# AlgoLab/RecGraph

Hardware: AMD Instinct MI355X
Metric: aligned reads/sec (-m 8 recombination, 1 kbp reads, 10k-row/32-path graph) (higher is better)
Workload: dtype int16

## Files before the change

### recgraph_amd/csrc/rg_host.hpp

```cpp
#pragma once
#include "rg_codes.hpp"

#include <atomic>
#include <cstdint>
#include <deque>
#include <functional>
#include <string>
#include <vector>

#include "../../include/recgraph_hip.h"

namespace rg {

extern thread_local std::string g_last_error;

#define RG_OPTIONS(X) \
    X(sweep_i32, "RG_SWEEP_I32", B, 0, 1, 0)           \
    X(three_sweeps, "RG_THREE_SWEEPS", B, 0, 1, 0)     \
    X(no_frec, "RG_NO_FREC", B, 0, 1, 0)               \
    X(debug, "RG_DEBUG", B, 0, 1, 0)                   \
    X(spin_wait, "RG_SPIN_WAIT", B, 0, 1, 0)           \
    X(no_gather, "RG_NO_GATHER", B, 0, 1, 0)           \
    X(no_split, "RG_NO_SPLIT", B, 0, 1, 0)             \
    X(no_spec, "RG_NO_SPEC", B, 0, 1, 0)               \
    X(spec_margin, "RG_SPEC_MARGIN", I, -(1 << 24), 1 << 24, 112)    \
    X(spec4_margin_x10, "RG_SPEC4_MARGIN_X10", I, 0, 1000, 25)       \
    X(stripe_c, "RG_STRIPE_C", I, 0, 32, 0)            \
    X(no_retire, "RG_NO_RETIRE", I, 0, 3, 0)           \
    X(retire_shift, "RG_RETIRE_SHIFT", I, 2, 12, RG_SWEEP16_RETIRE_SHIFT)    \
    X(no_order, "RG_NO_ORDER", B, 0, 1, 0)             \
    X(dsel_edge, "RG_DSEL_EDGE", I, 1, 1 << 20, 8)     \
    X(no_dsel, "RG_NO_DSEL", B, 0, 1, 0)               \
    X(no_pick2, "RG_NO_PICK2", B, 0, 1, 0)             \
    X(layer_i32, "RG_LAYER_I32", B, 0, 1, 0)           \
    X(lds_pad, "RG_LDS_PAD", I, 0, 40 << 10, 0)        \
    X(chunk_reads, "RG_CHUNK_READS", I, 0, 1 << 20, 0)    \
    X(launch_log, "RG_LAUNCH_LOG", B, 0, 1, 0)
struct Options {
#define RG_OPTION_FIELD(name, env, kind, lo, hi, def) std::atomic<int> name{def};
    RG_OPTIONS(RG_OPTION_FIELD)
#undef RG_OPTION_FIELD
};
struct OptionDesc {
    const char* name;
    const char* env;
    bool boolean;
    int lo, hi, def;
    std::atomic<int> Options::*slot;
};
extern const OptionDesc kOptionTable[];
extern const int kOptionCount;
const OptionDesc* find_option(const char* name);
void store_option(Options& o, const OptionDesc& d, long long value);
Options& options();
int wait_stream_sleeping(void* stream, void* ev, bool spin = false);

int fail(int code, const std::string& msg);

inline long long even_chunks(long long n, long long maxchunk) {
    const long long nchunks = (n + maxchunk - 1) / maxchunk;
    return (n + nchunks - 1) / nchunks;
}

// ... 135 lines not shown
```

### recgraph_amd/csrc/rg_kernel_timer.hpp

```cpp
#pragma once
#include <vector>

#include "rg_path_args.hpp"

namespace rg {

struct KernelTimer {
    hipStream_t stream = nullptr;
    bool spin = false;
    std::vector<hipEvent_t> ev;
    hipEvent_t done_ev = nullptr;
    std::vector<const char*> pend;
    std::vector<const char*> insts;

    KernelTimer() = default;
    KernelTimer(const KernelTimer&) = delete;
    ~KernelTimer() {
        for (auto e : ev) (void)hipEventDestroy(e);
        if (done_ev) (void)hipEventDestroy(done_ev);
    }
    void reset() { pend.clear(); insts.clear(); }
    int inst(const char* label, const char* what = "an untimed launch") {
        if (!label) return fail(RG_ERR_ARG, std::string("no kernel is compiled for this launch: ") + what);
        if (options().launch_log) insts.push_back(label);
        return RG_OK;
    }
    template <typename F>
    int run(const char* name, F&& launch) {
        const size_t used = 2 * pend.size();
        while (ev.size() < used + 2) {
            hipEvent_t e;
            HIPCHK(hipEventCreate(&e));
            ev.push_back(e);
        }
        HIPCHK(hipEventRecord(ev[used], stream));
        const char* label = launch();
        HIPCHK(hipGetLastError());
        HIPCHK(hipEventRecord(ev[used + 1], stream));
        pend.push_back(name);
        return inst(label, name);
    }
    int collect(KernelStats& stats) {
        if (!pend.empty()) {
            if (!done_ev) HIPCHK(hipEventCreateWithFlags(&done_ev, hipEventDisableTiming));
            HIPCHK((hipError_t)wait_stream_sleeping(stream, done_ev, spin));
            for (size_t k = 0; k < pend.size(); ++k) {
                float ms = 0;
                HIPCHK(hipEventElapsedTime(&ms, ev[2 * k], ev[2 * k + 1]));
                add_stat(stats, pend[k], ms, 1);
            }
            pend.clear();
        }
        for (const char* l : insts) add_stat(stats, std::string("inst:") + l, 0, 1);
        insts.clear();
        return RG_OK;
    }
};

}
```

### recgraph_amd/csrc/rg_path_driver.hip

```cpp
#include <algorithm>
#include <chrono>
#include <cstdio>
#include <cstdlib>
#include <cstring>

#include "gap/rg_path_gap.hpp"
#include "gap_local/rg_path_gap_local.hpp"
#include "rg_kernel_timer.hpp"
#include "rg_path_kernels.hpp"
#include "rg_path_plan.hpp"

namespace rg {

struct PathWorkImpl {
    bool tables = false;
    DevBuf<int> fpoff, fprow, fpslot, rpoff, rprow, rpslot;
    DevBuf<ReadState> state;
    DevBuf<int> roll, mf, wr, mfarg, wrarg, thr, flayer, rlayer;
    DevBuf<uint32_t> fdirs, rdirs, gdirs;
    DevBuf<Cand> fcand, rcand;
    DevBuf<unsigned> nf, nr, ridx, nrec, nrrec;
    DevBuf<int> frec, rrec;
    unsigned frec_cap = 0, rrec_cap = 0;
    DevBuf<int> lb;
// ... 299 lines not shown
        HIPCHK(hipMemsetAsync(w.nr.p, 0, sizeof(unsigned) * chunk, stream));
        ExpandArgs ea{w.state.p, w.frec.p, w.frec_cap, w.nrec.p, w.fcand.p, w.fcap, w.nf.p, w.wr.p, wpad, p.base_rec_cost, gd.knm, 0, off(), p.rec_band_width, p.scores[5]};
        RG_TRY(T.run("k_expand", [&] { return launch_expand(ea, chunk, plan.C, stream); }));
        ExpandArgs er{w.state.p, w.rrec.p, w.rrec_cap, w.nrrec.p, w.rcand.p, w.rcap, w.nr.p, w.mf.p, wpad, p.base_rec_cost, gd.knm, 1, off(), p.rec_band_width, p.scores[5]};
        RG_TRY(T.run("k_expand", [&] { return launch_expand(er, chunk, plan.C, stream); }));
    }
    SearchArgs sr{gd, w.state.p, w.fcand.p, w.rcand.p, w.nf.p, w.nr.p, w.ridx.p, w.fcap, w.rcap, w.wr.p, wpad, p.base_rec_cost, p.multi_rec_cost};
    RG_TRY(T.run("k_search", [&] { return launch_search(sr, chunk, stream); }));
    RG_TRY(T.inst(launch_need(w.state.p, w.nf.p, w.nr.p, plan.use_rec ? w.nrec.p : nullptr, plan.use_rec ? w.nrrec.p : nullptr, w.need.p, chunk, stream)));
    if (plan.spec) RG_TRY(T.inst(launch_verify(w.state.p, w.lb.p, w.need.p + 4, w.rt_flags.p, chunk, sa.dsel_pick, sa.dsel_pick2, sa.dsel_lo, sa.dsel_hi, stream)));
    return RG_OK;
}

int Run::enqueue_tail() {
    const int C = plan.C;
    LayerArgs la;
    memset(&la, 0, sizeof la);
    la.semi = plan.semi ? 1 : 0;
    la.nwv = plan.nwv;
    la.g = gd; la.sc = sc; la.reads = d_reads; la.read_off = off(); la.state = w.state.p; la.dir_words = plan.dir_words; la.dir_fmt = plan.use16 ? 1 : 0;
    la.layer_stride = plan.layer_stride; la.fpoff = w.fpoff.p; la.fprow = w.fprow.p; la.fpslot = w.fpslot.p;
    la.rpoff = w.rpoff.p; la.rprow = w.rprow.p; la.rpslot = w.rpslot.p;
    la.rev = 0; la.dirs = w.fdirs.p; la.dirs_stride = plan.fdirs_stride; la.layer = w.flayer.p;
    auto layer = [&]() { return plan.layer16 ? launch_layer16(la, chunk, C, stream) : launch_layer(la, chunk, C, stream); };
    RG_TRY(T.run("k_layer_fwd", layer));
    if (plan.mode == RG_MODE_RECOMBINATION) {
        la.rev = 1; la.dirs = w.rdirs.p; la.dirs_stride = plan.rdirs_stride; la.layer = w.rlayer.p;
        RG_TRY(T.run("k_layer_rev", layer));
    }
    TraceArgs ta;
    memset(&ta, 0, sizeof ta);
    ta.g = gd; ta.sc = sc; ta.reads = d_reads; ta.read_off = off(); ta.state = w.state.p; ta.rec = d_rec + done;
    ta.ops = d_ops + (long long)done * ops_stride; ta.ops_stride = ops_stride; ta.flayer = w.flayer.p;
    ta.rlayer = w.rlayer.p; ta.layer_stride = plan.layer_stride; ta.fpoff = w.fpoff.p; ta.fprow = w.fprow.p;
    ta.rpoff = w.rpoff.p; ta.rprow = w.rprow.p; ta.nreads = chunk; ta.mode = p.mode; ta.semi = plan.semi ? 1 : 0; ta.nwv = plan.nwv;
    RG_TRY(T.run("k_trace", [&] { return launch_trace(ta, C, stream); }));
    return read_back();
}

int Run::read_back() {
    HIPCHK(hipMemcpyAsync(w.h_sum, d_cells, sizeof(unsigned long long), hipMemcpyDeviceToHost, stream));
    HIPCHK(hipMemcpyAsync(w.h_sum + 5, d_cells + 1, sizeof(unsigned long long), hipMemcpyDeviceToHost, stream));
    HIPCHK(hipMemcpyAsync(w.h_sum + 1, w.need.p, 8 * sizeof(unsigned), hipMemcpyDeviceToHost, stream));
    return T.collect(stats);
}

int Run::enqueue_chunk() {
    HIPCHK(hipMemsetAsync(w.state.p, 0, sizeof(ReadState) * chunk, stream));
    if (plan.gap) return enqueue_pathwise_gap();
    SweepArgs sa = sweep_args();
    SeedArgs se;
    se.g = gd; se.state = w.state.p; se.nreads = chunk; se.mode = p.mode; se.sc = sc; se.reads = d_reads; se.read_off = off();
    int rc = plan.mode == RG_MODE_PATHWISE ? enqueue_pathwise(sa, se) : enqueue_recombination(sa, se);
    if (rc) return rc;
    return enqueue_tail();
}

int Run::dump_list_stats() {
    const unsigned* nd = need();
// ... 153 lines not shown
        const size_t per_read_all = plan.per_read_all(w.fcap, w.rcap, w.frec_cap, w.rrec_cap);
        int maxchunk = (int)std::min<size_t>(8192, std::max<size_t>(1, (budget >> oom_shift) / per_read_all));
        if (opt.chunk_reads > 0) maxchunk = std::min<int>(maxchunk, opt.chunk_reads);
        const double dbg_t0 = r.debug ? now_s() : 0;
        const int chunk = r.chunk = (int)even_chunks(nreads - r.done, maxchunk);
        bool oom = false;
        if ((rc = r.alloc_chunk(&oom))) {
            if (rc == RG_ERR_HIP && oom && chunk > 1 && oom_shift < 12) { ++oom_shift; continue; }
            return rc;
        }
        if (r.debug) fprintf(stderr, "[rg] chunk of %d reads: buffers ready after %.1f ms\n", chunk, (now_s() - dbg_t0) * 1e3);
        if ((rc = r.enqueue_chunk())) return rc;
        if (r.debug) fprintf(stderr, "[rg] chunk of %d reads: done after %.1f ms\n", chunk, (now_s() - dbg_t0) * 1e3);
        if (r.async_err != hipSuccess) return fail(RG_ERR_HIP, std::string("hipMemsetAsync: ") + hipGetErrorString(r.async_err));
        bool redo = false;
        if ((rc = r.regrow_lists(redo))) return rc;
        if (redo) continue;
        const unsigned long long chunk_cells = w.h_sum[0];
        cells_perf += w.h_sum[5];
        const unsigned nretry = r.nretry();
        if (r.debug && (plan.spec || plan.spec4)) fprintf(stderr, "[rg] speculative bound (margin %d): %u of %d reads did not reach it\n", plan.spec_margin, nretry, chunk);
        if (r.debug && plan.spec4 && nretry && (rc = r.dump_spec4_retries())) return rc;
        if (r.debug && plan.dsel && (rc = r.dump_dsel_retries())) return rc;
        if (nretry && (rc = r.second_pass(cells_perf))) return rc;
        cells_done += chunk_cells;
        r.done += chunk;
        add_stat(stats, "mem:work_bytes_per_read", (double)per_read_all, 1);
    }
    cells[0] += cells_done;
    cells[1] += cells_perf;
    return RG_OK;
}

}
```

### recgraph_amd/csrc/rg_path_kernels.hpp

```cpp
#pragma once
#include "rg_path_args.hpp"
#include "rg_path_plan.hpp"
#include "rg_launch_log.hpp"

namespace rg {

template <int H>
__device__ __forceinline__ void dir16_decode(unsigned w, unsigned& u16, unsigned& l16) {
    constexpr unsigned LOWH = (1u << H) - 1u;
    const unsigned t = __brev(w);
    u16 = ((t >> 24) & LOWH) | (((t >> 16) & LOWH) << H);
    l16 = ((t >> 8) & LOWH) | ((t & LOWH) << H);
}

struct SweepArgs {
    PathGraphDev g;
    DevScores sc;
    const uint8_t* reads;
    const long long* read_off;
    const uint8_t* bad;
    ReadState* state;
    int* roll;
    int rev;
    int track_best;
    const int* thr;
    const int4* fsteps;
// ... 127 lines not shown
    const int* wr;
    int wpad;
    int brc;
    float mrc;
};

struct LayerArgs {
    PathGraphDev g;
    DevScores sc;
    const uint8_t* reads;
    const long long* read_off;
    ReadState* state;
    int rev;
    const uint32_t* dirs;
    long long dirs_stride;
    int dir_words;
    int dir_fmt;
    int semi;
    int* layer;
    long long layer_stride;
    const int* fpoff; const int* fprow; const int* fpslot;
    const int* rpoff; const int* rprow; const int* rpslot;
    int nwv;
};

struct TraceArgs {
    PathGraphDev g;
    DevScores sc;
    const uint8_t* reads;
    const long long* read_off;
    ReadState* state;
    DevRecord* rec;
    uint8_t* ops;
    long long ops_stride;
    const int* flayer;
    const int* rlayer;
    long long layer_stride;
    const int* fpoff; const int* fprow;
    const int* rpoff; const int* rprow;
    int nreads;
    int mode;
    int semi;
    int nwv;
};

const char* launch_sweep(const SweepArgs& a, int nreads, int C, hipStream_t s);
const char* launch_sweep16(const SweepArgs& a, int nreads, int C, hipStream_t s);
const char* launch_expand(const ExpandArgs& a, int nreads, int C, hipStream_t s);
const char* launch_colmax_rec(const ExpandArgs& a, int* colmax_out, int* colarg_out, int nreads, int C, hipStream_t s);
const char* launch_seed(const SeedArgs& a, hipStream_t s);
const char* launch_opt0(const Opt0Args& a, int nreads, int C, hipStream_t s);
const char* launch_opt0_16(const Opt0Args& a, int nreads, int C, hipStream_t s);
const char* launch_pick(const PickArgs& a, int nreads, hipStream_t s);
const char* launch_order(const int* pick, const int* pick2, int* order, int nreads, hipStream_t s);
const char* launch_verify4(ReadState* st, const int* lb, unsigned* nretry, uint8_t* flags, int nreads, const int* dsel_pick, hipStream_t s);
const char* launch_verify(ReadState* st, const int* lb, unsigned* nretry, uint8_t* flags, int nreads, const int* dsel_pick, const int* dsel_pick2, int dsel_lo, int dsel_hi, hipStream_t s);
const char* launch_gather_reads(const uint8_t* reads, const long long* off, const int* idx, const long long* sub_off, uint8_t* out, int n, hipStream_t s);
const char* launch_scatter_results(const int* idx, const DevRecord* sub_rec, const uint8_t* sub_ops, DevRecord* rec, uint8_t* ops, long long ops_stride, int n, hipStream_t s);
const char* launch_threshold(const ThrArgs& a, int nreads, hipStream_t s);
const char* launch_bound(const BoundArgs& a, int nreads, hipStream_t s);
const char* launch_search(const SearchArgs& a, int nreads, hipStream_t s);
const char* launch_need(const ReadState* st, const unsigned* nf, const unsigned* nr, const unsigned* nrec, const unsigned* nrrec,
                 unsigned* need, int nreads, hipStream_t s);
const char* launch_layer(const LayerArgs& a, int nreads, int C, hipStream_t s);
const char* launch_layer16(const LayerArgs& a, int nreads, int C, hipStream_t s);
const char* launch_trace(const TraceArgs& a, int C, hipStream_t s);

}
```

### recgraph_amd/csrc/rg_path_plan.cpp

```cpp
#include "rg_path_plan.hpp"

#include <algorithm>
#include <climits>
#include <cmath>
#include <cstdlib>
#include <cstring>
#include <mutex>

namespace rg {

#define RG_OPTION_ROW(name, env, kind, lo, hi, def) {#name, env, #kind[0] == 'B', lo, hi, def, &Options::name},
const OptionDesc kOptionTable[] = {RG_OPTIONS(RG_OPTION_ROW)};
#undef RG_OPTION_ROW
const int kOptionCount = (int)(sizeof kOptionTable / sizeof kOptionTable[0]);

const OptionDesc* find_option(const char* name) {
    if (!name) return nullptr;
    for (const OptionDesc& d : kOptionTable)
        if (!strcmp(name, d.name)) return &d;
    return nullptr;
}
void store_option(Options& o, const OptionDesc& d, long long value) {
    o.*d.slot = d.boolean ? (value ? 1 : 0) : (int)std::max<long long>(d.lo, std::min<long long>(value, d.hi));
}
Options& options() {
    static Options o;
    static std::once_flag once;
    std::call_once(once, [] {
        for (const OptionDesc& d : kOptionTable) {
            const char* v = getenv(d.env);
            if (!v) continue;
            store_option(o, d, d.boolean ? (*v && strcmp(v, "0") != 0) : atoi(v));
        }
    });
    return o;
// ... 96 lines not shown
        o.gaps_nonpos = o.gaps_nonpos && p.scores[x * 6 + 5] <= 0 && p.scores[5 * 6 + x] <= 0;
        o.gaps_agree = o.gaps_agree && p.scores[5 * 6 + x] == p.scores[x * 6 + 5];
        for (int y = 0; y < 5; ++y) o.maxmatch = std::max(o.maxmatch, p.scores[x * 6 + y]);
    }
    o.two_sweep = recomb && o.gaps_nonpos && !opt.three_sweeps;
    o.use_rec = o.two_sweep && use16 && !opt.no_frec;
    const bool paths_ok = P <= 64 || use16;
    o.spec = o.two_sweep && spec_level < 2 && !semi && paths_ok && !opt.no_spec;
    o.score_scale = std::max(1, o.maxmatch / 2);
    const int per_kbp = (max_n + 999) / 1000;
    o.spec_margin = ((nwv > 1 ? opt.spec_margin * per_kbp : (int)opt.spec_margin) + (spec_level == 1 ? 320 * per_kbp : 0)) *
                    (opt.spec_margin > 0 ? o.score_scale : 1);
    o.pick_two = o.spec && !opt.no_pick2;
    o.dsel = o.spec && o.use_rec && spec_level == 0 && !opt.no_dsel;
    { const int e = L / std::max(1, (int)opt.dsel_edge); o.dsel_lo = e; o.dsel_hi = L - 1 - e; }
    o.rec_pen = p.base_rec_cost + (int)std::ceil(p.multi_rec_cost * 8.0f);
    o.spec4 = o.mode == RG_MODE_PATHWISE && !semi && use16 && o.gaps_nonpos && spec_level == 0 && !opt.no_spec;
    o.spec4_margin = o.spec_margin * opt.spec4_margin_x10 / 10;
    o.retire4 = o.spec4 && opt.no_retire != 1;
    o.dsel4 = o.spec4 && !opt.no_dsel;
    o.order = !opt.no_order;
    o.opt16 = use16;
    o.layer16 = use16 && o.gaps_agree && !opt.layer_i32;
    o.gather_ok = use16 && !opt.no_gather;
    o.use_split = o.gather_ok && !semi && C <= 16 && !opt.no_split;
    o.retire = (use16 || nwv == 1 || C <= 16) && paths_ok && !semi && recomb && o.gaps_nonpos && opt.no_retire != 1;
    o.retire_fwd = o.retire && opt.no_retire != 3;
    o.retire_rev = o.retire && opt.no_retire != 2;
    o.fcap = (o.two_sweep && !o.use_rec) ? 1u << 20 : 1u << 15;
    o.rcap = o.use_rec ? 1u << 16 : 1u << 19;
    o.frec_cap = o.spec ? 1u << 14 : 1u << 16;
    o.rrec_cap = o.spec ? 1u << 13 : 1u << 15;
    return RG_OK;
}

void build_path_rows(const HostGraph& h, bool fwd, std::vector<int>& poff, std::vector<int>& prow, std::vector<int>& pslot) {
    const std::vector<int32_t>& goff = fwd ? h.fgoff : h.rgoff;
    const std::vector<GroupDesc>& groups = fwd ? h.fgroups : h.rgroups;
    const int P = h.P, L = h.L;
    std::vector<std::vector<std::pair<int, int>>> per(P);
    for (int step = 1; step + 1 < L; ++step) {
        const int i = fwd ? step : L - 1 - step;
        for (int gi = goff[i]; gi < goff[i + 1]; ++gi)
            for (int b = 0; b < 64; ++b)
                if ((groups[gi].mask >> b) & 1) per[groups[gi].page * 64 + b].push_back({i, groups[gi].slot});
    }
// ... 40 lines not shown
```

### recgraph_amd/csrc/rg_path_plan.hpp

```cpp
#pragma once
#include <cstddef>
#include <vector>

#include "rg_host.hpp"

namespace rg {

struct ReadState {
    uint32_t status;
    int s0;
    int seed_path;
    int end_row;
    int end_row_best;
    int fwd_path, rev_path, fen, rsn, rec_col, displacement;
    float fscore;
    int bound;
    int sink_val[RG_MAXP];
    int trace_score;
    int path_end_row[RG_MAXP];
};

struct Cand {
    int row, col, val, path;
};

struct PathPlanInput {
    int P, L, fslots, rslots, max_path_rows, max_n;
};

struct PathPlan {
    int C, nwv, wpad, dir_words, recw;
    long long layer_stride, fdirs_stride, rdirs_stride;
    size_t per_read;
    int mode;
    bool semi;
    int maxmatch;
    bool gaps_nonpos;
    bool gaps_agree;
    int score_scale;
    bool use16;
    bool two_sweep, use_rec, spec, pick_two, dsel, spec4, opt16, layer16;
    bool retire, use_split, gather_ok;
    bool retire_fwd, retire_rev;
    bool retire4, dsel4;
    bool order;
    int spec_margin, spec4_margin, dsel_lo, dsel_hi, rec_pen;
    unsigned fcap, rcap, frec_cap, rrec_cap;
    bool gap;
    bool local;
    int gap_words;
    long long gdirs_stride;

    size_t per_read_all(unsigned fcap_, unsigned rcap_, unsigned frec_cap_, unsigned rrec_cap_) const {
        if (mode != RG_MODE_RECOMBINATION) return per_read;
        return per_read + (size_t)fcap_ * sizeof(Cand) + (size_t)rcap_ * (sizeof(Cand) + 4) +
               (use_rec ? (size_t)(frec_cap_ + rrec_cap_) * recw * 4 : 0);
    }
};

int plan_pathwise(const rg_params& p, const PathPlanInput& in, const Options& opt, int spec_level, PathPlan& out);

bool sweep16_admissible(const DevScores& sc, int max_path_rows, int max_n, int C);

void build_path_rows(const HostGraph& h, bool fwd, std::vector<int>& poff, std::vector<int>& prow, std::vector<int>& pslot);
// ... 5 lines not shown
```

### recgraph_amd/csrc/rg_pathwise.hip

```cpp
#include "rg_path_kernels.hpp"

namespace rg {

constexpr int NEG = INT32_MIN / 4;
#ifndef RG_SWEEP_WAVES
#define RG_SWEEP_WAVES 2
#endif

struct Rows {
    int* base;
    __device__ __forceinline__ int ld(int k, int idx, int wpad) const { return base[(long long)k * wpad + idx]; }
    __device__ __forceinline__ void st(int k, int idx, int wpad, int v) const { base[(long long)k * wpad + idx] = v; }
};
extern __shared__ __attribute__((aligned(16))) int g_lds[];

__device__ __forceinline__ int wave_excl_max(int v, int lane) {
    (void)lane;
    return dpp_shr1(dpp_incl_max(v, NEG), NEG);
}

constexpr int FIFO_WORDS = 128;
struct StripeFifo {
    volatile int* buf;
    unsigned* head;
// ... 1183 lines not shown
            const int l = (q == 0 ? nk : cur[q - 1]) + gl[q];
            const int mx = max(max(d, u), l);
            const uint32_t code = mx == d ? 1u : (mx == u ? 2u : 3u);
            tw[q / 16] |= code << (2 * (q % 16));
        }
        tdir[(long long)(t + 1) * a.dir_words + wv * dww + wl] = tw[0];
        if (C > 16) tdir[(long long)(t + 1) * a.dir_words + wv * dww + WAVE + wl] = tw[C <= 16 ? 0 : 1];
        if (!rev && irow == start_row) {
            int v = 0;
#pragma unroll
            for (int q = 0; q < C; ++q) if (q == start_col % C) v = cur[q];
            if (lane == start_col / C) rs->trace_score = v;
        }
        if (recomb && irow == (rev ? rs->rsn : rs->fen)) break;
    }
}

template <int C>
__global__ __launch_bounds__(64) void k_trace(TraceArgs a) {
    const int rd = blockIdx.x * blockDim.x + threadIdx.x;
    if (rd >= a.nreads) return;
    ReadState* rs = a.state + rd;
    DevRecord* rec = a.rec + rd;
    if (rs->status & (ST_BAD_BASE | ST_WOULD_PANIC | ST_OVERFLOW | ST_RETRY)) {
        rec->status = rs->status & ~ST_RETRY; rec->n_ops = 0; rec->n_fwd_ops = 0; rec->score = 0;
        return;
    }
    const long long ro = a.read_off[rd];
    const int n = (int)(a.read_off[rd + 1] - ro);
    uint8_t* ops = a.ops + (long long)rd * a.ops_stride;
    int nops = 0;
    const bool recomb = (a.mode == RG_MODE_RECOMBINATION || a.mode == RG_MODE_RECOMBINATION_SEMI) && rs->fwd_path != rs->rev_path;
    const int dww = WAVE * (C <= 16 ? 1 : 2);
    const int dw = dww * a.nwv;
    auto move = [&](const uint32_t* td, int idx, int c) -> uint32_t {
        const int q = c % C, gl = c / C;
        return (td[(long long)idx * dw + (gl / WAVE) * dww + (q / 16) * WAVE + gl % WAVE] >> (2 * (q % 16))) & 3u;
    };
    const uint32_t* fl = reinterpret_cast<const uint32_t*>(a.flayer) + (long long)rd * a.layer_stride;
    const int fp = rs->fwd_path;
    const int fbeg = a.fpoff[fp], fnr = a.fpoff[fp + 1] - fbeg;
    int start_row = recomb ? rs->fen : rs->end_row;
    int j = recomb ? rs->rec_col : n;
    int lo = 0, hi = fnr - 1, idx = -1;
    while (lo <= hi) { int mid = (lo + hi) >> 1; int r = a.fprow[fbeg + mid]; if (r == start_row) { idx = mid; break; } if (r < start_row) lo = mid + 1; else hi = mid - 1; }
    if (idx < 0) { rec->status = ST_WOULD_PANIC; rec->n_ops = 0; return; }
    int t = idx + 1;
    const int score = rs->trace_score;
    while (t > 0 && j > 0) {
        const uint32_t mv = move(fl, t, j);
        if (mv == 1u) { ops[nops++] = OP_D; t -= 1; j -= 1; }
        else if (mv == 2u) { ops[nops++] = OP_U; t -= 1; }
        else { ops[nops++] = OP_L; j -= 1; }
    }
    while (j > 0) { ops[nops++] = OP_L; j -= 1; }
    while (!a.semi && t > 0) { ops[nops++] = OP_U; t -= 1; }
    const int nfwd = nops;
    if (recomb) {
        const int rp = rs->rev_path;
        const uint32_t* rl = reinterpret_cast<const uint32_t*>(a.rlayer) + (long long)rd * a.layer_stride;
        const int rbeg = a.rpoff[rp], rnr = a.rpoff[rp + 1] - rbeg;
        int lo2 = 0, hi2 = rnr - 1, ridx = -1;
        while (lo2 <= hi2) { int mid = (lo2 + hi2) >> 1; int r = a.rprow[rbeg + mid]; if (r == rs->rsn) { ridx = mid; break; } if (r > rs->rsn) lo2 = mid + 1; else hi2 = mid - 1; }
        if (ridx < 0) { rec->status = ST_WOULD_PANIC; rec->n_ops = 0; return; }
        int tt = ridx + 1;
        int jj = rs->rec_col;
        while (tt > 0 && jj < n) {
            const uint32_t mv = move(rl, tt, n - jj);
            if (mv == 1u) { ops[nops++] = OP_D; tt -= 1; jj += 1; }
            else if (mv == 2u) { ops[nops++] = OP_U; tt -= 1; }
            else { ops[nops++] = OP_L; jj += 1; }
        }
        while (jj < n) { ops[nops++] = OP_L | OP_CONT; jj += 1; }
        while (!a.semi && tt > 0) { ops[nops++] = OP_U | OP_CONT; tt -= 1; }
    }
    rec->status = rs->status;
    rec->score = score;
    rec->fscore = rs->fscore;
    rec->end_row = start_row;
    rec->end_col = n;
    rec->stop_row = 0; rec->stop_col = 0;
    rec->best_path = fp;
    rec->rev_path = recomb ? rs->rev_path : fp;
    rec->fen = rs->fen; rec->rsn = rs->rsn; rec->rec_col = rs->rec_col; rec->displacement = rs->displacement;
    rec->n_ops = nops; rec->n_fwd_ops = nfwd;
}

__global__ __launch_bounds__(256) void k_need(const ReadState* st, const unsigned* nf, const unsigned* nr, const unsigned* nrec,
                                              const unsigned* nrrec, unsigned* need, int nreads) {
    const int rd = blockIdx.x * blockDim.x + threadIdx.x;
    unsigned v[4] = {0, 0, 0, 0};
    if (rd < nreads && !(st[rd].status & (ST_BAD_BASE | ST_WOULD_PANIC))) {
        v[0] = nf[rd]; v[1] = nr[rd];
        if (nrec) v[2] = nrec[rd];
        if (nrrec) v[3] = nrrec[rd];
    }
#pragma unroll
    for (int e = 0; e < 4; ++e) {
        for (int d = WAVE / 2; d >= 1; d >>= 1) v[e] = max(v[e], (unsigned)__shfl_xor((int)v[e], d, WAVE));
// ... 120 lines not shown
```

### recgraph_amd/csrc/rg_sweep16.hip

```cpp
#include <algorithm>
#include <type_traits>

#include "rg_path_kernels.hpp"

namespace rg {

namespace {

constexpr int NEG32 = INT32_MIN / 4;
constexpr int NEG16 = -30000;
constexpr int NEGPAIR = (int)(((unsigned)(NEG16 & 0xffff) << 16) | (unsigned)(NEG16 & 0xffff));
constexpr int ONE2 = 0x00010001;

typedef unsigned u32x4 __attribute__((ext_vector_type(4)));
typedef unsigned u32x2 __attribute__((ext_vector_type(2)));
__device__ __forceinline__ __amdgpu_buffer_rsrc_t uniform_rsrc(const void* base, unsigned bytes) {
    const unsigned long long u = (unsigned long long)base;
    const unsigned lo = (unsigned)__builtin_amdgcn_readfirstlane((int)(unsigned)u), hi = (unsigned)__builtin_amdgcn_readfirstlane((int)(unsigned)(u >> 32));
    void* p = (void*)(((unsigned long long)hi << 32) | lo);
    return __builtin_amdgcn_make_buffer_rsrc(p, 0, (int)__builtin_amdgcn_readfirstlane((int)bytes), 0x00020000);
}
typedef short s16x2 __attribute__((ext_vector_type(2)));
typedef unsigned short u16x2 __attribute__((ext_vector_type(2)));

// ... 1375 lines not shown
        colarg_out[(long long)rd * a.wpad + j] = b ? (int)(((unsigned)b << 8) | ((unsigned)key & 255u)) : 0;
    }
}

const char* launch_colmax_rec(const ExpandArgs& a, int* colmax_out, int* colarg_out, int nreads, int C, hipStream_t s) {
    const size_t bytes = (size_t)a.wpad * sizeof(unsigned long long);
    switch (C) {
        case 4: RG_LAUNCH(k_colmax_rec, (4), dim3(nreads), dim3(256), bytes, s, a, colmax_out, colarg_out);
        case 8: RG_LAUNCH(k_colmax_rec, (8), dim3(nreads), dim3(256), bytes, s, a, colmax_out, colarg_out);
        case 16: RG_LAUNCH(k_colmax_rec, (16), dim3(nreads), dim3(256), bytes, s, a, colmax_out, colarg_out);
        default: RG_LAUNCH(k_colmax_rec, (32), dim3(nreads), dim3(256), bytes, s, a, colmax_out, colarg_out);
    }
}


template <int C>
__global__ __launch_bounds__(64, C <= 16 ? LAYER16_WAVES : 1) void k_layer16(LayerArgs a) {
    constexpr int H = C / 2;
    const int rd = blockIdx.x;
    const int lane = threadIdx.x;
    const PathGraphDev& g = a.g;
    ReadState* rs = a.state + rd;
    if (rs->status & (ST_BAD_BASE | ST_WOULD_PANIC | ST_OVERFLOW | ST_RETRY)) return;
    const bool rev = a.rev;
    const int path = rev ? rs->rev_path : rs->fwd_path;
    const bool recomb = rs->fwd_path != rs->rev_path;
    if (rev && !recomb) return;
    const long long ro = a.read_off[rd];
    const int n = (int)(a.read_off[rd + 1] - ro);
    const uint8_t* read = a.reads + ro - 1;
    const int ncols = rev ? n : n + 1;
    const int GAP = 5;
    extern __shared__ __attribute__((aligned(16))) int lds16[];
    int* sct = lds16;
    int* s2 = lds16 + 64;
    int* sprof = s2 + 5 * 64;
    if (lane < 36) sct[lane] = a.sc.t[lane];
    __syncthreads();
    const int gcost = __builtin_amdgcn_readfirstlane(sct[GAP]);
    for (int e = lane; e < 5 * 64; e += WAVE) {
        const int li = e >> 6, cl = e & 7, ch = (e >> 3) & 7;
        s2[e] = (cl < 6 && ch < 6) ? pack16(sct[li * 6 + cl] - gcost, sct[li * 6 + ch] - gcost) : 0;
    }
    __syncthreads();
    int cur[H];
#pragma unroll
// ... 275 lines not shown
```

Measured before the change: 124,400.

## Add banded layer-window kernel for path layers with full-width fallback

```diff
diff --git a/recgraph_amd/csrc/layer_window/rg_layer_window.hip b/recgraph_amd/csrc/layer_window/rg_layer_window.hip
--- /dev/null
+++ b/recgraph_amd/csrc/layer_window/rg_layer_window.hip
@@ -0,0 +1,264 @@
+#include "rg_layer_window.hpp"
+
+#include "../rg_path_kernels.hpp"
+
+namespace rg {
+
+namespace {
+
+constexpr int UNK = LAYER_WINDOW_UNKNOWN;
+constexpr int UNKPAIR = (int)(((unsigned)(UNK & 0xffff) << 16) | (unsigned)(UNK & 0xffff));
+constexpr int KNOWNPAIR = (int)(((unsigned)(LAYER_WINDOW_KNOWN & 0xffff) << 16) | (unsigned)(LAYER_WINDOW_KNOWN & 0xffff));
+constexpr int ONE2 = 0x00010001;
+
+typedef short s16x2 __attribute__((ext_vector_type(2)));
+
+__device__ __forceinline__ int pk_add(int a, int b) {
+    return __builtin_bit_cast(int, (s16x2)(__builtin_bit_cast(s16x2, a) + __builtin_bit_cast(s16x2, b)));
+}
+__device__ __forceinline__ int pk_sub(int a, int b) {
+    return __builtin_bit_cast(int, (s16x2)(__builtin_bit_cast(s16x2, a) - __builtin_bit_cast(s16x2, b)));
+}
+__device__ __forceinline__ int pk_max(int a, int b) {
+    return __builtin_bit_cast(int, __builtin_elementwise_max(__builtin_bit_cast(s16x2, a), __builtin_bit_cast(s16x2, b)));
+}
+__device__ __forceinline__ int pk_min(int a, int b) {
+    return __builtin_bit_cast(int, __builtin_elementwise_min(__builtin_bit_cast(s16x2, a), __builtin_bit_cast(s16x2, b)));
+}
+__device__ __forceinline__ int pk_sub_sat(int a, int b) {
+    return __builtin_bit_cast(int, __builtin_elementwise_sub_sat(__builtin_bit_cast(s16x2, a), __builtin_bit_cast(s16x2, b)));
+}
+__device__ __forceinline__ int pk_sign(int v) {
+    return __builtin_bit_cast(int, (s16x2)(__builtin_bit_cast(s16x2, v) >> (s16x2)(15)));
+}
+__device__ __forceinline__ int pack16(int lo, int hi) { return (int)(((unsigned)hi << 16) | ((unsigned)lo & 0xffffu)); }
+__device__ __forceinline__ int lo16(int v) { return (int)(short)(v & 0xffff); }
+__device__ __forceinline__ int hi16(int v) { return v >> 16; }
+__device__ __forceinline__ int bfi(int mask, int a, int b) { return __builtin_amdgcn_bitop3_b32(mask, a, b, 0xCA); }
+__device__ __forceinline__ int left_lane(int v, int edge, int fill) {
+    int r = __builtin_amdgcn_update_dpp(v, v, 0x13C, 0xf, 0xf, false);
+    asm volatile("" : "+v"(r));
+    return bfi(edge, fill, r);
+}
+
+}
+
+template <int C, int CW>
+__global__ __launch_bounds__(64, 8) void k_layer_win(LayerArgs a) {
+    static_assert(CW == 2 || CW == 4, "a column block is half a byte or a byte of the layer buffer");
+    static_assert(C == 4 || C == 8 || C == 16, "packed rows, one direction word per lane and row");
+    constexpr int H = CW / 2;
+    constexpr int W = WAVE * CW;
+    constexpr int WPAD = WAVE * C;
+    constexpr int NBLK = WPAD / CW;
+    constexpr unsigned LOWH = (1u << H) - 1u;
+    constexpr unsigned FULL = (LOWH << 16) | LOWH;
+    const int rd = blockIdx.x;
+    const int lane = threadIdx.x;
+    const PathGraphDev& g = a.g;
+    ReadState* rs = a.state + rd;
+    if (rs->status & (ST_BAD_BASE | ST_WOULD_PANIC | ST_OVERFLOW | ST_RETRY | ST_LAYER_FULL)) return;
+    const bool rev = a.rev;
+    const int path = rev ? rs->rev_path : rs->fwd_path;
+    const bool recomb = rs->fwd_path != rs->rev_path;
+    if (rev && !recomb) return;
+    const long long ro = a.read_off[rd];
+    const int n = (int)(a.read_off[rd + 1] - ro);
+    const uint8_t* read = a.reads + ro - 1;
+    const int ncols = rev ? n : n + 1;
+    const int GAP = 5;
+    __shared__ int sct[64];
+    __shared__ int s2[5 * 64];
+    __shared__ int kkp[NBLK];
+    if (lane < 36) sct[lane] = a.sc.t[lane];
+    __syncthreads();
+    const int gcost = __builtin_amdgcn_readfirstlane(sct[GAP]);
+    for (int e = lane; e < 5 * 64; e += WAVE) {
+        const int li = e >> 6, cl = e & 7, ch = (e >> 3) & 7;
+        s2[e] = (cl < 6 && ch < 6) ? pack16(sct[li * 6 + cl] - gcost, sct[li * 6 + ch] - gcost) : 0;
+    }
+    auto code = [&](int c) -> int { return (c >= 1 && c < ncols) ? (int)(rev ? read[n - c + 1] : read[c]) : 4; };
+    for (int b = lane; b < NBLK; b += WAVE) {
+        int kk = 0;
+#pragma unroll
+        for (int r = 0; r < H; ++r) kk |= (code(b * CW + r) | (code(b * CW + H + r) << 3)) << (8 * r);
+        kkp[b] = kk;
+    }
+    __syncthreads();
+    const int* prow = rev ? a.rprow : a.fprow;
+    const int* pslot = rev ? a.rpslot : a.fpslot;
+    const int* poff = rev ? a.rpoff : a.fpoff;
+    const int pbase = poff[path];
+    const int nrows = poff[path + 1] - pbase;
+    const int start_row = rev ? rs->rsn : (recomb ? rs->fen : rs->end_row);
+    const int start_col = rev ? n - rs->rec_col : (recomb ? rs->rec_col : n);
+    const int sidx = __builtin_amdgcn_readfirstlane(layer_row_index(prow + pbase, nrows, start_row, rev));
+    if (sidx < 0) return;
+    const int t_start = sidx + 1;
+    uint8_t* tdir = reinterpret_cast<uint8_t*>(reinterpret_cast<uint32_t*>(a.layer) + (long long)rd * a.layer_stride);
+    const uint32_t* dirs = a.dirs + (long long)rd * a.dirs_stride;
+    auto block_of = [&](int lbk) -> int { return lbk + ((lane - lbk) & (WAVE - 1)); };
+    int lbk = layer_window_left(start_col, t_start, 0, W, WPAD) / CW;
+    int blk = block_of(lbk);
+    int kk = kkp[blk];
+    int cur[H];
+#pragma unroll
+    for (int r = 0; r < H; ++r) {
+        const int c0 = blk * CW + r, c1 = c0 + H;
+        cur[r] = pack16(c0 < ncols ? 0 : UNK, c1 < ncols ? 0 : UNK);
+    }
+    constexpr int PF = 2;
+    int pf_li[PF];
+    uint32_t pf_w[PF];
+    int nx_row = -1, nx_slot = 0;
+    auto fetch_idx = [&](int tt) {
+        nx_row = -1; nx_slot = 0;
+        if (tt <= sidx) { nx_row = prow[pbase + tt]; nx_slot = pslot[pbase + tt]; }
+    };
+    auto prefetch = [&](int tt, int& li_o, uint32_t& w_o) {
+        li_o = 4; w_o = 0;
+        if (nx_row >= 0) {
+            const int b = block_of(layer_window_left(start_col, t_start, tt + 1, W, WPAD) / CW);
+            li_o = g.lnz[nx_row];
+            w_o = dirs[(long long)nx_slot * a.dir_words + (b * CW) / C];
+        }
+    };
+#pragma unroll
+    for (int k = 0; k < PF; ++k) { fetch_idx(k); prefetch(k, pf_li[k], pf_w[k]); }
+    fetch_idx(PF);
+    const int g_i = gcost;
+    const int g0 = a.semi ? 0 : g_i;
+    const int GI = pack16(g_i, g_i);
+    for (int t = 0; t <= sidx; ++t) {
+        const int li = pf_li[0];
+        const uint32_t word = pf_w[0];
+#pragma unroll
+        for (int k = 0; k + 1 < PF; ++k) { pf_li[k] = pf_li[k + 1]; pf_w[k] = pf_w[k + 1]; }
+        prefetch(t + PF, pf_li[PF - 1], pf_w[PF - 1]);
+        fetch_idx(t + PF + 1);
+        const int nlbk = layer_window_left(start_col, t_start, t + 1, W, WPAD) / CW;
+        if (nlbk != lbk) {
+            lbk = nlbk;
+            const int nb = block_of(lbk);
+            const int nkk = kkp[nb];
+            if (nb != blk) {
+                kk = nkk;
+#pragma unroll
+                for (int r = 0; r < H; ++r) cur[r] = UNKPAIR;
+            }
+            blk = nb;
+        }
+        const int p = lbk & (WAVE - 1);
+        const int pos = (lane - p) & (WAVE - 1);
+        const int edge = pos == 0 ? -1 : 0;
+        const int GI0 = blk == 0 ? pack16(g0, g_i) : GI;
+        unsigned u16, l16;
+        dir16_decode<C / 2>(word, u16, l16);
+        const int q0 = (blk * CW) & (C - 1);
+        const unsigned ub = u16 >> q0, lb = l16 >> q0;
+        const unsigned um2 = (ub & LOWH) | (((ub >> H) & LOWH) << 16);
+        const unsigned lm2 = (lb & LOWH) | (((lb >> H) & LOWH) << 16);
+        int s[H], MU[H], ML[H];
+#pragma unroll
+        for (int r = 0; r < H; ++r) {
+            s[r] = s2[li * 64 + ((kk >> (8 * r)) & 63)];
+            MU[r] = pk_sub(0, (int)((um2 >> r) & (unsigned)ONE2));
+            ML[r] = pk_sub(0, (int)((lm2 >> r) & (unsigned)ONE2));
+        }
+        const unsigned long long have = __ballot(lm2 != FULL);
+        const unsigned long long rot = p ? ((have >> p) | (have << (WAVE - p))) : have;
+        const unsigned long long below = rot & ((1ull << pos) - 1ull);
+        const int src = below ? ((63 - __clzll((long long)below) + p) & (WAVE - 1)) : -1;
+        int old[H];
+#pragma unroll
+        for (int r = 0; r < H; ++r) old[r] = cur[r];
+        int o1 = __builtin_amdgcn_alignbit(old[H - 1], left_lane(old[H - 1], edge, UNKPAIR), 16);
+        {
+            int prev = o1, lastv = UNKPAIR;
+#pragma unroll
+            for (int r = 0; r < H; ++r) {
+                const int base = pk_add(bfi(MU[r], old[r], prev), bfi(MU[r], r == 0 ? GI0 : GI, s[r]));
+                cur[r] = base;
+                lastv = bfi(ML[r], lastv, base);
+                prev = old[r];
+            }
+            const unsigned nl = ~lm2 & FULL;
+            const int v_lo = lo16(lastv), v_hi = hi16(lastv);
+            const int zl = (nl >> 16) ? v_hi : ((nl & 0xffffu) ? v_lo : UNK);
+            const int fetched = __shfl(zl, src < 0 ? lane : src, WAVE);
+            const int bl = src < 0 ? UNK : max(fetched, UNK);
+            const int bh = (nl & 0xffffu) ? max(v_lo, UNK) : bl;
+            int vprev = pack16(bl, bh);
+#pragma unroll
+            for (int r = 0; r < H; ++r) {
+                int v = bfi(ML[r], vprev, cur[r]);
+                v = bfi(pk_sign(pk_sub_sat(v, KNOWNPAIR)), UNKPAIR, v);
+                cur[r] = v;
+                vprev = v;
+            }
+        }
+        const bool zero_prev = rev && t == 0 && path != 0;
+        if (zero_prev) {
+#pragma unroll
+            for (int r = 0; r < H; ++r) {
+                const int c0 = blk * CW + r, c1 = c0 + H;
+                old[r] = pack16(-c0 * gcost, -c1 * gcost);
+            }
+            o1 = __builtin_amdgcn_alignbit(old[H - 1], left_lane(old[H - 1], edge, UNKPAIR), 16);
+            if (blk == 0) o1 = pack16(gcost, hi16(o1));
+        }
+        int nl = __builtin_amdgcn_alignbit(cur[H - 1], left_lane(cur[H - 1], edge, UNKPAIR), 16);
+        unsigned tw = 0;
+#pragma unroll
+        for (int r = 0; r < H; ++r) {
+            const int d = pk_add(o1, s[r]);
+            const int u = pk_add(old[r], GI);
+            const int mx = pk_max(pk_max(d, u), nl);
+            const int unk = pk_sign(pk_sub_sat(pk_min(pk_min(d, u), nl), KNOWNPAIR));
+            const int nd = pk_sign(pk_sub_sat(d, mx));
+            const int nu = pk_sign(pk_sub_sat(u, mx));
+            const int b0 = __builtin_amdgcn_bitop3_b32(nd, nu, ONE2, 0x8A);
+            const unsigned code2 = (unsigned)((b0 | (nd & 0x00020002)) & ~unk);
+            tw |= code2 << (2 * r);
+            o1 = old[r];
+            nl = cur[r];
+        }
+        const unsigned codes = (tw & ((1u << (2 * H)) - 1u)) | ((tw >> 16) << (2 * H));
+        const int c0 = blk * CW;
+        uint8_t* out = tdir + (long long)(t + 1) * a.dir_words * 4 + ((c0 / C) * 4 + ((c0 & (C - 1)) >> 2));
+        if constexpr (CW == 4) {
+            *out = (uint8_t)codes;
+        } else {
+            const unsigned other = (unsigned)__builtin_amdgcn_update_dpp(0, (int)codes, 0xF5, 0xf, 0xf, false);
+            if (!(lane & 1)) *out = (uint8_t)(codes | (other << 4));
+        }
+        if (t == sidx && !rev) {
+            const int q = start_col & (CW - 1);
+            int pv = 0;
+#pragma unroll
+            for (int r = 0; r < H; ++r) if (r == q % H) pv = cur[r];
+            const int z = q >= H ? hi16(pv) : lo16(pv);
+            if (blk == start_col / CW) {
+                if (z < LAYER_WINDOW_KNOWN) atomicOr(&rs->status, ST_LAYER_FULL);
+                else rs->trace_score = z + start_col * gcost;
+            }
+        }
+    }
+}
+
+const char* launch_layer_window(const LayerArgs& a, int nreads, int C, int window, hipStream_t s) {
+    if (window == LAYER_WINDOW_NARROW) {
+        switch (C) {
+            case 4: RG_LAUNCH(k_layer_win, (4, 2), dim3(nreads), dim3(64), 0, s, a);
+            case 8: RG_LAUNCH(k_layer_win, (8, 2), dim3(nreads), dim3(64), 0, s, a);
+            default: RG_LAUNCH(k_layer_win, (16, 2), dim3(nreads), dim3(64), 0, s, a);
+        }
+    }
+    switch (C) {
+        case 4: RG_LAUNCH(k_layer_win, (4, 4), dim3(nreads), dim3(64), 0, s, a);
+        case 8: RG_LAUNCH(k_layer_win, (8, 4), dim3(nreads), dim3(64), 0, s, a);
+        default: RG_LAUNCH(k_layer_win, (16, 4), dim3(nreads), dim3(64), 0, s, a);
+    }
+}
+
+}
diff --git a/recgraph_amd/csrc/layer_window/rg_layer_window.hpp b/recgraph_amd/csrc/layer_window/rg_layer_window.hpp
--- /dev/null
+++ b/recgraph_amd/csrc/layer_window/rg_layer_window.hpp
@@ -0,0 +1,44 @@
+#pragma once
+#include <stdint.h>
+
+#if defined(__HIPCC__)
+#define RG_LW_HD __host__ __device__ inline __attribute__((always_inline))
+#else
+#define RG_LW_HD inline
+#endif
+
+namespace rg {
+
+constexpr uint32_t ST_LAYER_FULL = 0x400u;
+constexpr int NEED_LAYER_FULL = 5;
+
+constexpr const char* LAYER_WINDOW_LOG = "mem:layer_window:";
+
+constexpr int LAYER_WINDOW_DEFAULT = 256;
+constexpr int LAYER_WINDOW_NARROW = 128;
+
+RG_LW_HD int layer_window_left(int start_col, int t_start, int t, int W, int wpad) {
+    int e = start_col - (t_start - t) - W / 2;
+    const int hi = wpad - W;
+    e = e > hi ? hi : e;
+    e = e < 0 ? 0 : e;
+    return e & ~3;
+}
+
+RG_LW_HD int layer_row_index(const int* list, int nr, int row, bool descending) {
+    int lo = 0, hi = nr - 1;
+    while (lo <= hi) {
+        const int mid = (lo + hi) >> 1;
+        const int r = list[mid];
+        if (r == row) return mid;
+        if (descending ? r > row : r < row) lo = mid + 1;
+        else hi = mid - 1;
+    }
+    return -1;
+}
+
+constexpr int LAYER_WINDOW_UNKNOWN = -30000;
+constexpr int LAYER_WINDOW_KNOWN = -27000;
+constexpr int LAYER_WINDOW_ZLO = -24000;
+
+}
diff --git a/recgraph_amd/csrc/rg_host.hpp b/recgraph_amd/csrc/rg_host.hpp
--- a/recgraph_amd/csrc/rg_host.hpp
+++ b/recgraph_amd/csrc/rg_host.hpp
@@ -36,9 +36,12 @@
     X(lds_pad, "RG_LDS_PAD", I, 0, 40 << 10, 0)        \
     X(chunk_reads, "RG_CHUNK_READS", I, 0, 1 << 20, 0)    \
     X(launch_log, "RG_LAUNCH_LOG", B, 0, 1, 0)
+#define RG_TUNING_OPTIONS(Y) \
+    Y(layer_window, "RG_LAYER_WINDOW", I, 0, 256, 256)
 struct Options {
 #define RG_OPTION_FIELD(name, env, kind, lo, hi, def) std::atomic<int> name{def};
     RG_OPTIONS(RG_OPTION_FIELD)
+    RG_TUNING_OPTIONS(RG_OPTION_FIELD)
 #undef RG_OPTION_FIELD
 };
 struct OptionDesc {
diff --git a/recgraph_amd/csrc/rg_kernel_timer.hpp b/recgraph_amd/csrc/rg_kernel_timer.hpp
--- a/recgraph_amd/csrc/rg_kernel_timer.hpp
+++ b/recgraph_amd/csrc/rg_kernel_timer.hpp
@@ -1,4 +1,5 @@
 #pragma once
+#include <utility>
 #include <vector>
 
 #include "rg_path_args.hpp"
@@ -11,7 +12,7 @@
     std::vector<hipEvent_t> ev;
     hipEvent_t done_ev = nullptr;
     std::vector<const char*> pend;
-    std::vector<const char*> insts;
+    std::vector<std::pair<const char*, const char*>> insts;
 
     KernelTimer() = default;
     KernelTimer(const KernelTimer&) = delete;
@@ -20,13 +21,13 @@
         if (done_ev) (void)hipEventDestroy(done_ev);
     }
     void reset() { pend.clear(); insts.clear(); }
-    int inst(const char* label, const char* what = "an untimed launch") {
+    int inst(const char* label, const char* what = "an untimed launch", const char* family = "inst:", bool always = false) {
         if (!label) return fail(RG_ERR_ARG, std::string("no kernel is compiled for this launch: ") + what);
-        if (options().launch_log) insts.push_back(label);
+        if (always || options().launch_log) insts.push_back({family, label});
         return RG_OK;
     }
     template <typename F>
-    int run(const char* name, F&& launch) {
+    int run(const char* name, F&& launch, const char* family = "inst:", bool always = false) {
         const size_t used = 2 * pend.size();
         while (ev.size() < used + 2) {
             hipEvent_t e;
@@ -38,7 +39,7 @@
         HIPCHK(hipGetLastError());
         HIPCHK(hipEventRecord(ev[used + 1], stream));
         pend.push_back(name);
-        return inst(label, name);
+        return inst(label, name, family, always);
     }
     int collect(KernelStats& stats) {
         if (!pend.empty()) {
@@ -51,7 +52,7 @@
             }
             pend.clear();
         }
-        for (const char* l : insts) add_stat(stats, std::string("inst:") + l, 0, 1);
+        for (const auto& l : insts) add_stat(stats, std::string(l.first) + l.second, 0, 1);
         insts.clear();
         return RG_OK;
     }
diff --git a/recgraph_amd/csrc/rg_path_driver.hip b/recgraph_amd/csrc/rg_path_driver.hip
--- a/recgraph_amd/csrc/rg_path_driver.hip
+++ b/recgraph_amd/csrc/rg_path_driver.hip
@@ -345,11 +345,18 @@
     la.layer_stride = plan.layer_stride; la.fpoff = w.fpoff.p; la.fprow = w.fprow.p; la.fpslot = w.fpslot.p;
     la.rpoff = w.rpoff.p; la.rprow = w.rprow.p; la.rpslot = w.rpslot.p;
     la.rev = 0; la.dirs = w.fdirs.p; la.dirs_stride = plan.fdirs_stride; la.layer = w.flayer.p;
-    auto layer = [&]() { return plan.layer16 ? launch_layer16(la, chunk, C, stream) : launch_layer(la, chunk, C, stream); };
-    RG_TRY(T.run("k_layer_fwd", layer));
+    const int win = plan.layer_window;
+    auto layer = [&]() {
+        if (win) return launch_layer_window(la, chunk, C, win, stream);
+        return plan.layer16 ? launch_layer16(la, chunk, C, stream) : launch_layer(la, chunk, C, stream);
+    };
+    auto fwd_side = [&]() { la.rev = 0; la.dirs = w.fdirs.p; la.dirs_stride = plan.fdirs_stride; la.layer = w.flayer.p; };
+    auto rev_side = [&]() { la.rev = 1; la.dirs = w.rdirs.p; la.dirs_stride = plan.rdirs_stride; la.layer = w.rlayer.p; };
+    const char* family = win ? LAYER_WINDOW_LOG : "inst:";
+    RG_TRY(T.run("k_layer_fwd", layer, family, win != 0));
     if (plan.mode == RG_MODE_RECOMBINATION) {
-        la.rev = 1; la.dirs = w.rdirs.p; la.dirs_stride = plan.rdirs_stride; la.layer = w.rlayer.p;
-        RG_TRY(T.run("k_layer_rev", layer));
+        rev_side();
+        RG_TRY(T.run("k_layer_rev", layer, family, win != 0));
     }
     TraceArgs ta;
     memset(&ta, 0, sizeof ta);
@@ -357,7 +364,19 @@
     ta.ops = d_ops + (long long)done * ops_stride; ta.ops_stride = ops_stride; ta.flayer = w.flayer.p;
     ta.rlayer = w.rlayer.p; ta.layer_stride = plan.layer_stride; ta.fpoff = w.fpoff.p; ta.fprow = w.fprow.p;
     ta.rpoff = w.rpoff.p; ta.rprow = w.rprow.p; ta.nreads = chunk; ta.mode = p.mode; ta.semi = plan.semi ? 1 : 0; ta.nwv = plan.nwv;
+    ta.window = win; ta.nfull = w.need.p + NEED_LAYER_FULL;
     RG_TRY(T.run("k_trace", [&] { return launch_trace(ta, C, stream); }));
+    if (win) {
+        la.only_full = 1;
+        fwd_side();
+        RG_TRY(T.run("k_layer_full", [&] { return launch_layer16(la, chunk, C, stream); }));
+        if (plan.mode == RG_MODE_RECOMBINATION) {
+            rev_side();
+            RG_TRY(T.run("k_layer_full", [&] { return launch_layer16(la, chunk, C, stream); }));
+        }
+        ta.window = 0; ta.only_full = 1;
+        RG_TRY(T.run("k_trace_full", [&] { return launch_trace(ta, C, stream); }));
+    }
     return read_back();
 }
 
@@ -557,6 +576,10 @@
         if (r.debug && (plan.spec || plan.spec4)) fprintf(stderr, "[rg] speculative bound (margin %d): %u of %d reads did not reach it\n", plan.spec_margin, nretry, chunk);
         if (r.debug && plan.spec4 && nretry && (rc = r.dump_spec4_retries())) return rc;
         if (r.debug && plan.dsel && (rc = r.dump_dsel_retries())) return rc;
+        if (plan.layer_window) {
+            add_stat(stats, "mem:layer_full_reads", (double)r.need()[NEED_LAYER_FULL], 1);
+            if (r.debug) fprintf(stderr, "[rg] layer window of %d columns: %u of %d reads took the full-width layers\n", plan.layer_window, r.need()[NEED_LAYER_FULL], chunk);
+        }
         if (nretry && (rc = r.second_pass(cells_perf))) return rc;
         cells_done += chunk_cells;
         r.done += chunk;
diff --git a/recgraph_amd/csrc/rg_path_kernels.hpp b/recgraph_amd/csrc/rg_path_kernels.hpp
--- a/recgraph_amd/csrc/rg_path_kernels.hpp
+++ b/recgraph_amd/csrc/rg_path_kernels.hpp
@@ -2,6 +2,7 @@
 #include "rg_path_args.hpp"
 #include "rg_path_plan.hpp"
 #include "rg_launch_log.hpp"
+#include "layer_window/rg_layer_window.hpp"
 
 namespace rg {
 
@@ -175,6 +176,7 @@
     const int* fpoff; const int* fprow; const int* fpslot;
     const int* rpoff; const int* rprow; const int* rpslot;
     int nwv;
+    int only_full;
 };
 
 struct TraceArgs {
@@ -195,6 +197,9 @@
     int mode;
     int semi;
     int nwv;
+    int window;
+    int only_full;
+    unsigned* nfull;
 };
 
 const char* launch_sweep(const SweepArgs& a, int nreads, int C, hipStream_t s);
@@ -218,5 +223,6 @@
 const char* launch_layer(const LayerArgs& a, int nreads, int C, hipStream_t s);
 const char* launch_layer16(const LayerArgs& a, int nreads, int C, hipStream_t s);
 const char* launch_trace(const TraceArgs& a, int C, hipStream_t s);
+const char* launch_layer_window(const LayerArgs& a, int nreads, int C, int window, hipStream_t s);
 
 }
diff --git a/recgraph_amd/csrc/rg_path_plan.cpp b/recgraph_amd/csrc/rg_path_plan.cpp
--- a/recgraph_amd/csrc/rg_path_plan.cpp
+++ b/recgraph_amd/csrc/rg_path_plan.cpp
@@ -10,7 +10,7 @@
 namespace rg {
 
 #define RG_OPTION_ROW(name, env, kind, lo, hi, def) {#name, env, #kind[0] == 'B', lo, hi, def, &Options::name},
-const OptionDesc kOptionTable[] = {RG_OPTIONS(RG_OPTION_ROW)};
+const OptionDesc kOptionTable[] = {RG_OPTIONS(RG_OPTION_ROW) RG_TUNING_OPTIONS(RG_OPTION_ROW)};
 #undef RG_OPTION_ROW
 const int kOptionCount = (int)(sizeof kOptionTable / sizeof kOptionTable[0]);
 
@@ -153,6 +153,15 @@
     o.order = !opt.no_order;
     o.opt16 = use16;
     o.layer16 = use16 && o.gaps_agree && !opt.layer_i32;
+    o.layer_window = 0;
+    if (o.layer16 && C <= 16 && spec_level == 0 && opt.layer_window >= LAYER_WINDOW_NARROW) {
+        long long smin = INT32_MAX;
+        for (int x = 0; x < 5; ++x)
+            for (int y = 0; y < 5; ++y) smin = std::min<long long>(smin, p.scores[x * 6 + y]);
+        const long long g = p.scores[5];
+        const long long zlo = (long long)(in.max_path_rows + 2) * g - (long long)(max_n + 2) * std::max(0ll, g - smin);
+        if (zlo >= LAYER_WINDOW_ZLO) o.layer_window = opt.layer_window >= LAYER_WINDOW_DEFAULT ? LAYER_WINDOW_DEFAULT : LAYER_WINDOW_NARROW;
+    }
     o.gather_ok = use16 && !opt.no_gather;
     o.use_split = o.gather_ok && !semi && C <= 16 && !opt.no_split;
     o.retire = (use16 || nwv == 1 || C <= 16) && paths_ok && !semi && recomb && o.gaps_nonpos && opt.no_retire != 1;
diff --git a/recgraph_amd/csrc/rg_path_plan.hpp b/recgraph_amd/csrc/rg_path_plan.hpp
--- a/recgraph_amd/csrc/rg_path_plan.hpp
+++ b/recgraph_amd/csrc/rg_path_plan.hpp
@@ -3,6 +3,7 @@
 #include <vector>
 
 #include "rg_host.hpp"
+#include "layer_window/rg_layer_window.hpp"
 
 namespace rg {
 
@@ -40,6 +41,7 @@
     int score_scale;
     bool use16;
     bool two_sweep, use_rec, spec, pick_two, dsel, spec4, opt16, layer16;
+    int layer_window;
     bool retire, use_split, gather_ok;
     bool retire_fwd, retire_rev;
     bool retire4, dsel4;
diff --git a/recgraph_amd/csrc/rg_pathwise.hip b/recgraph_amd/csrc/rg_pathwise.hip
--- a/recgraph_amd/csrc/rg_pathwise.hip
+++ b/recgraph_amd/csrc/rg_pathwise.hip
@@ -1229,10 +1229,16 @@
     if (rd >= a.nreads) return;
     ReadState* rs = a.state + rd;
     DevRecord* rec = a.rec + rd;
+    if (a.only_full) {
+        if (!(rs->status & ST_LAYER_FULL)) return;
+        rs->status &= ~ST_LAYER_FULL;
+    }
     if (rs->status & (ST_BAD_BASE | ST_WOULD_PANIC | ST_OVERFLOW | ST_RETRY)) {
-        rec->status = rs->status & ~ST_RETRY; rec->n_ops = 0; rec->n_fwd_ops = 0; rec->score = 0;
+        rec->status = rs->status & ~(ST_RETRY | ST_LAYER_FULL); rec->n_ops = 0; rec->n_fwd_ops = 0; rec->score = 0;
         return;
     }
+    auto give_up = [&]() { rs->status |= ST_LAYER_FULL; atomicAdd(a.nfull, 1u); };
+    if (a.window && (rs->status & ST_LAYER_FULL)) { atomicAdd(a.nfull, 1u); return; }
     const long long ro = a.read_off[rd];
     const int n = (int)(a.read_off[rd + 1] - ro);
     uint8_t* ops = a.ops + (long long)rd * a.ops_stride;
@@ -1240,8 +1246,12 @@
     const bool recomb = (a.mode == RG_MODE_RECOMBINATION || a.mode == RG_MODE_RECOMBINATION_SEMI) && rs->fwd_path != rs->rev_path;
     const int dww = WAVE * (C <= 16 ? 1 : 2);
     const int dw = dww * a.nwv;
-    auto move = [&](const uint32_t* td, int idx, int c) -> uint32_t {
+    auto move = [&](const uint32_t* td, int idx, int c, int t0, int c0) -> uint32_t {
         const int q = c % C, gl = c / C;
+        if (a.window) {
+            const int left = layer_window_left(c0, t0, idx, a.window, C * WAVE);
+            if (c < left || c >= left + a.window) return 0u;
+        }
         return (td[(long long)idx * dw + (gl / WAVE) * dww + (q / 16) * WAVE + gl % WAVE] >> (2 * (q % 16))) & 3u;
     };
     const uint32_t* fl = reinterpret_cast<const uint32_t*>(a.flayer) + (long long)rd * a.layer_stride;
@@ -1254,11 +1264,13 @@
     if (idx < 0) { rec->status = ST_WOULD_PANIC; rec->n_ops = 0; return; }
     int t = idx + 1;
     const int score = rs->trace_score;
+    const int ft0 = t, fc0 = j;
     while (t > 0 && j > 0) {
-        const uint32_t mv = move(fl, t, j);
+        const uint32_t mv = move(fl, t, j, ft0, fc0);
         if (mv == 1u) { ops[nops++] = OP_D; t -= 1; j -= 1; }
         else if (mv == 2u) { ops[nops++] = OP_U; t -= 1; }
-        else { ops[nops++] = OP_L; j -= 1; }
+        else if (mv == 3u || !a.window) { ops[nops++] = OP_L; j -= 1; }
+        else { give_up(); return; }
     }
     while (j > 0) { ops[nops++] = OP_L; j -= 1; }
     while (!a.semi && t > 0) { ops[nops++] = OP_U; t -= 1; }
@@ -1272,16 +1284,18 @@
         if (ridx < 0) { rec->status = ST_WOULD_PANIC; rec->n_ops = 0; return; }
         int tt = ridx + 1;
         int jj = rs->rec_col;
+        const int rt0 = tt, rc0 = n - jj;
         while (tt > 0 && jj < n) {
-            const uint32_t mv = move(rl, tt, n - jj);
+            const uint32_t mv = move(rl, tt, n - jj, rt0, rc0);
             if (mv == 1u) { ops[nops++] = OP_D; tt -= 1; jj += 1; }
             else if (mv == 2u) { ops[nops++] = OP_U; tt -= 1; }
-            else { ops[nops++] = OP_L; jj += 1; }
+            else if (mv == 3u || !a.window) { ops[nops++] = OP_L; jj += 1; }
+            else { give_up(); return; }
         }
         while (jj < n) { ops[nops++] = OP_L | OP_CONT; jj += 1; }
         while (!a.semi && tt > 0) { ops[nops++] = OP_U | OP_CONT; tt -= 1; }
     }
-    rec->status = rs->status;
+    rec->status = rs->status & ~ST_LAYER_FULL;
     rec->score = score;
     rec->fscore = rs->fscore;
     rec->end_row = start_row;
diff --git a/recgraph_amd/csrc/rg_sweep16.hip b/recgraph_amd/csrc/rg_sweep16.hip
--- a/recgraph_amd/csrc/rg_sweep16.hip
+++ b/recgraph_amd/csrc/rg_sweep16.hip
@@ -1421,6 +1421,7 @@
     const PathGraphDev& g = a.g;
     ReadState* rs = a.state + rd;
     if (rs->status & (ST_BAD_BASE | ST_WOULD_PANIC | ST_OVERFLOW | ST_RETRY)) return;
+    if (a.only_full && !(rs->status & ST_LAYER_FULL)) return;
     const bool rev = a.rev;
     const int path = rev ? rs->rev_path : rs->fwd_path;
     const bool recomb = rs->fwd_path != rs->rev_path;
```

Result: faster. 127,800 (median of 6 runs) (+2.7%).
